# mpkuse/solve_keyframe_pose_graph

Measured on AMD Instinct MI355X. Metric: LM iters/sec + final chi2 vs Ceres, 100k-pose/300k-edge SE(3) graph, higher is better.
Workload: dtype f64

## Files before the change

solve_keyframe_pose_graph_amd/csrc/pgo_handle.hpp:

```cpp
#pragma once
#include <hip/hip_runtime.h>

#include <chrono>
#include <cstdlib>
#include <cstring>
#include <memory>
#include <string>
#include <thread>
#include <vector>

#include "pgo.h"
#include "pgo_internal.hpp"
#include "pgo_comm.hpp"
#include "pgo_mg_host.hpp"

#pragma GCC visibility push(hidden)
namespace pgo {

inline double now_s() { return std::chrono::duration<double>(std::chrono::steady_clock::now().time_since_epoch()).count(); }

inline bool debug_hooks_enabled() { static const bool on = []() { const char* e = std::getenv("PGO_ENABLE_DEBUG_HOOKS"); return e && e[0] == '1' && e[1] == 0; }(); return on; }
inline bool debug_poison() { static const bool on = []() { const char* e = std::getenv("PGO_DEBUG_POISON"); return debug_hooks_enabled() && e && e[0] == '1' && e[1] == 0; }(); return on; }
inline bool debug_break_coarse() { if (!debug_hooks_enabled()) return false; const char* e = std::getenv("PGO_DEBUG_BREAK_COARSE"); return e && e[0] == '1' && e[1] == 0; }

inline bool debug_no_split_update() { static const bool on = []() { const char* e = std::getenv("PGO_DEBUG_NO_SPLIT_UPDATE"); return debug_hooks_enabled() && e && e[0] == '1' && e[1] == 0; }(); return on; }
inline bool debug_split_hosts(int* a, int* b) {
    static const int v = []() {
        const char* e = std::getenv("PGO_DEBUG_SPLIT_HOSTS");
        if (!debug_hooks_enabled() || !e) return -1;
        char* end = nullptr; const long x = std::strtol(e, &end, 10);
        if (!end || *end != ',' || x < 0 || x > 63) return -1;
        const long y = std::strtol(end + 1, &end, 10);
        return (end && *end == 0 && y >= x && y <= 63) ? (int)(x * 64 + y) : -1;
    }();
    if (v < 0) return false;
    *a = v / 64; *b = v % 64;
    return true;
}

inline int debug_graph_after() {
    static const int v = []() {
        const char* e = std::getenv("PGO_DEBUG_GRAPH_AFTER");
        if (!debug_hooks_enabled() || !e) return 192;
        char* end = nullptr; const long n = std::strtol(e, &end, 10);
        return (end && *end == 0 && n >= 2 && n <= 1000000 && (n & 1) == 0) ? (int)n : 192;
    }();
    return v;
}

template <class T>
struct DBuf {
    T* p = nullptr;
    size_t cap = 0;
    DBuf() = default;
    DBuf(const DBuf&) = delete;
    DBuf& operator=(const DBuf&) = delete;
    ~DBuf() { if (p) (void)hipFree(p); }
    hipError_t ensure(size_t n) {
        if (n <= cap) return hipSuccess;
        if (p) { (void)hipFree(p); p = nullptr; cap = 0; }
        const size_t want = n + n / 8 + 64;
        hipError_t e = hipMalloc((void**)&p, want * sizeof(T));
        if (e == hipSuccess) cap = want;
        if (e == hipSuccess && debug_poison()) { e = hipMemset(p, 0xFF, want * sizeof(T)); if (e == hipSuccess) e = hipDeviceSynchronize(); }
        return e;
    }
    hipError_t upload(const std::vector<T>& v, hipStream_t st) {
        hipError_t e = ensure(v.empty() ? 1 : v.size());
        if (e == hipSuccess && !v.empty()) e = hipMemcpyAsync(p, v.data(), v.size() * sizeof(T), hipMemcpyHostToDevice, st);
        return e;
    }
};

struct EventPair {
    hipEvent_t e0 = nullptr, e1 = nullptr;
    hipError_t create() { hipError_t e = hipEventCreate(&e0); if (e == hipSuccess) e = hipEventCreate(&e1); return e; }
    ~EventPair() { if (e0) (void)hipEventDestroy(e0); if (e1) (void)hipEventDestroy(e1); }
};

struct HostClass {
    std::vector<int32_t> c1, c2, sw;
    std::vector<double> meas;
    std::vector<double> loss;
    int64_t size() const { return (int64_t)c1.size(); }
};

struct MgPrepared;
struct MgPreparedFree { void operator()(MgPrepared* Q) const; };
using MgImage = std::unique_ptr<MgPrepared, MgPreparedFree>;

struct LevelPlanDev { const int32_t* send_idx = nullptr; const int32_t* recv_idx = nullptr; const pgo_mg::ExchangePlan* plan = nullptr; };
struct SetupPlanDev { const int32_t* val_send = nullptr; const int32_t* val_dst = nullptr; const int32_t* val_sum_ptr = nullptr; const int32_t* val_sum_src = nullptr;
                      const int32_t* ps_send = nullptr; const int32_t* ps_recv = nullptr; const int32_t* rv_send = nullptr; const int32_t* rv_recv = nullptr; };
struct OwnRange { int64_t row0 = 0, row1 = 0, blk0 = 0, blk1 = 0, ps0 = 0, ps1 = 0, w0 = 0, w1 = 0, rT0 = 0, rT1 = 0; };

struct MgJob {
    enum Kind { none, fresh, regroup };
    Kind kind = none;
    std::thread thread;
    MgImage out;
    int rc = 0;
    MgImage old;
};

struct MgState {
    DBuf<double> f64; DBuf<int32_t> i32; DBuf<int64_t> i64;
    MgDev M{}; MgLevelDev levels[MG_MAX_LEVELS];
    bool fine = false; MgLevelDev fineF{}, fineT{};
    int fine_auto = -1;
    bool built = false, active = false;
    pgo_mg::BuildCache cache;
    std::vector<double> sw_built;
    int regroups = 0;
    uint64_t geometry_epoch = 0;
    MgJob job;
    std::vector<LevelPlanDev> lvl_plan;
    std::vector<pgo_mg::ExchangePlan> plans;
    std::vector<uint8_t> dist;
    pgo_mg::SetupPlans setup; int first_whole = 0;
    int32_t fw_row0 = 0, fw_row1 = 0; int64_t fw_blk0 = 0, fw_blk1 = 0;
    std::vector<SetupPlanDev> su_plan;
// ... 222 lines not shown
```

solve_keyframe_pose_graph_amd/csrc/pgo_kernels.hip:

```cpp
#include <algorithm>

#include "pgo_internal.hpp"

namespace pgo {

#ifndef PGO_NO_UNIFORM
__device__ __forceinline__ int wave_in_grid() { return __builtin_amdgcn_readfirstlane((int)(((int64_t)blockIdx.x * blockDim.x + threadIdx.x) >> 6)); }
__device__ __forceinline__ int wave_in_block() { return __builtin_amdgcn_readfirstlane((int)(threadIdx.x >> 6)); }
#else
__device__ __forceinline__ int wave_in_grid() { return (int)(((int64_t)blockIdx.x * blockDim.x + threadIdx.x) >> 6); }
__device__ __forceinline__ int wave_in_block() { return (int)(threadIdx.x >> 6); }
#endif

__device__ __forceinline__ double wave_sum(double v) {
#pragma unroll
    for (int o = 32; o > 0; o >>= 1) v += __shfl_down(v, o, 64);
    return v;
}
__device__ __forceinline__ double wave_max(double v) {
#pragma unroll
    for (int o = 32; o > 0; o >>= 1) v = fmax(v, __shfl_down(v, o, 64));
    return v;
}
#ifndef PGO_SERIAL_HEAD
__device__ __forceinline__ double strided_share(const double* __restrict__ p, int n) {
    constexpr int MAXK = 12;
    double v[MAXK];
#pragma unroll
    for (int k = 0; k < MAXK; ++k) { const int i = (int)threadIdx.x + k * (int)blockDim.x; v[k] = i < n ? p[i] : 0.0; }
    double s = 0.0;
#pragma unroll
    for (int k = 0; k < MAXK; ++k) s += v[k];
    for (int i = (int)threadIdx.x + MAXK * (int)blockDim.x; i < n; i += blockDim.x) s += p[i];
    return s;
}
#else
__device__ __forceinline__ double strided_share(const double* __restrict__ p, int n) { double s = 0.0; for (int i = threadIdx.x; i < n; i += blockDim.x) s += p[i]; return s; }
#endif
__device__ __forceinline__ double block_sum(double v, double* buf) {
    const int lane = threadIdx.x & 63, wave = threadIdx.x >> 6, nw = (blockDim.x + 63) >> 6;
    v = wave_sum(v);
    __syncthreads();
    if (lane == 0) buf[wave] = v;
    __syncthreads();
    double s = 0.0;
    if (threadIdx.x == 0) for (int i = 0; i < nw; ++i) s += buf[i];
    return s;
}
__device__ __forceinline__ double block_total(const double* __restrict__ partials, int n, double* buf) {
    double v = strided_share(partials, n);
    const int lane = threadIdx.x & 63, wave = threadIdx.x >> 6, nw = (blockDim.x + 63) >> 6;
    v = wave_sum(v);
    __syncthreads();
    if (lane == 0) buf[wave] = v;
    __syncthreads();
    double s = 0.0;
    for (int i = 0; i < nw; ++i) s += buf[i];
    return s;
}

__device__ __forceinline__ int pm(int r, int c) { return (c >> 1) * 12 + r * 2 + (c & 1); }

__device__ __forceinline__ void block_total2(const double* __restrict__ pa, int na, const double* __restrict__ pb, int nb, double* buf , double& sa, double& sb) {
    double va = strided_share(pa, na), vb = strided_share(pb, nb);
    const int lane = threadIdx.x & 63, wave = threadIdx.x >> 6, nw = (blockDim.x + 63) >> 6;
    va = wave_sum(va); vb = wave_sum(vb);
    __syncthreads();
    if (lane == 0) { buf[wave] = va; buf[nw + wave] = vb; }
    __syncthreads();
    sa = 0.0; sb = 0.0;
    for (int i = 0; i < nw; ++i) { sa += buf[i]; sb += buf[nw + i]; }
}

__device__ __forceinline__ void block_total3(const double* __restrict__ pa, int na, const double* __restrict__ pb, int nb, const double* __restrict__ pc, int nc, double* buf ,
                                             double& sa, double& sb, double& sc) {
    double va = strided_share(pa, na), vb = strided_share(pb, nb), vc = strided_share(pc, nc);
    const int lane = threadIdx.x & 63, wave = threadIdx.x >> 6, nw = (blockDim.x + 63) >> 6;
    va = wave_sum(va); vb = wave_sum(vb); vc = wave_sum(vc);
    __syncthreads();
    if (lane == 0) { buf[wave] = va; buf[nw + wave] = vb; buf[2 * nw + wave] = vc; }
    __syncthreads();
    sa = 0.0; sb = 0.0; sc = 0.0;
    for (int i = 0; i < nw; ++i) { sa += buf[i]; sb += buf[nw + i]; sc += buf[2 * nw + i]; }
// ... 1026 lines not shown
    return (int)g;
}
__global__ void cg_set_tolerance_kernel(CgDev C, double tol2) {
    if (threadIdx.x == 0 && blockIdx.x == 0) { C.scal[3] = tol2; if (!C.flags[1]) C.flags[0] = 0; }
}
void launch_cg_set_tolerance(const CgDev& C, double tol2, hipStream_t st) { hipLaunchKernelGGL(cg_set_tolerance_kernel, dim3(1), dim3(64), 0, st, C, tol2); }
__global__ void cg_poll_kernel(CgDev C, int32_t* __restrict__ hflags, double* __restrict__ hscal) {
    if (threadIdx.x < 3) { hflags[threadIdx.x] = C.flags[threadIdx.x]; hscal[threadIdx.x] = C.scal[threadIdx.x]; }
}
void launch_cg_poll(const CgDev& C, int32_t* host_flags, double* host_scal, hipStream_t st) { hipLaunchKernelGGL(cg_poll_kernel, dim3(1), dim3(64), 0, st, C, host_flags, host_scal); }

void launch_cg_init(const GraphDev& G, const CgDev& C, int warm, double tol2, hipStream_t st) {
    const int g = cg_grid(G);
    hipLaunchKernelGGL(cg_init_kernel, dim3(g), dim3(CG_BLOCK), 0, st, G, C, warm);
    hipLaunchKernelGGL(cg_scalars_init_kernel, dim3(1), dim3(256), 0, st, C, g, g, tol2);
}
void launch_cg_init_scalars(const CgDev& C, int nparts, int nparts_bb, double tol2, hipStream_t st) { hipLaunchKernelGGL(cg_scalars_init_kernel, dim3(1), dim3(256), 0, st, C, nparts, nparts_bb, tol2); }
int launch_cg_init_vectors(const GraphDev& G, const CgDev& C, int warm, hipStream_t st) {
    const int g = cg_grid(G);
    hipLaunchKernelGGL(cg_init_kernel, dim3(g), dim3(CG_BLOCK), 0, st, G, C, warm);
    return g;
}
void launch_cg_spmv(const GraphDev& G, const CgDev& C, int k, double tol2, hipStream_t st) {
    const int g = cg_grid(G);
    hipLaunchKernelGGL(cg_spmv_kernel, dim3(g), dim3(CG_BLOCK), 0, st, G, C, k & 1, k == 0 ? 1 : 0, g, tol2);
}
void launch_cg_update(const GraphDev& G, const CgDev& C, int k, int n_pq_partials, hipStream_t st) {
    const int g = cg_grid(G);
    hipLaunchKernelGGL(cg_update_kernel<false>, dim3(g), dim3(CG_BLOCK), 0, st, G, C, k & 1, n_pq_partials, g, 0);
}
void launch_cg_update_sr(const GraphDev& G, const CgDev& C, int k, int first, int n_pq_partials, hipStream_t st) {
    const int g = cg_grid(G);
    hipLaunchKernelGGL(cg_update_kernel<true>, dim3(g), dim3(CG_BLOCK), 0, st, G, C, k & 1, n_pq_partials, g, first);
}
void launch_cgcg_dots(const GraphDev& G, const CgDev& C, hipStream_t st) { hipLaunchKernelGGL(cgcg_dots_kernel, dim3(cg_grid(G)), dim3(CG_BLOCK), 0, st, G, C); }
void launch_cg_reduce2_live(const CgDev& C, const double* pa, int na, const double* pb, int nb, double* out, hipStream_t st) {
    hipLaunchKernelGGL(cg_reduce2_live_kernel, dim3(1), dim3(256), 0, st, C, pa, na, pb, nb, out);
}
void launch_cgcg_update(const GraphDev& G, const CgDev& C, int k, int first, hipStream_t st, const double* xq, const int32_t* sh_of, const double* two) {
    hipLaunchKernelGGL(cgcg_update_kernel, dim3(cg_grid(G)), dim3(CG_BLOCK), 0, st, G, C, k & 1, first, xq, sh_of, two);
}
void launch_cgcg_scalars_init(const CgDev& C, const double* bb_src, double tol2, hipStream_t st) { hipLaunchKernelGGL(cgcg_scalars_init_kernel, dim3(1), dim3(64), 0, st, C, bb_src, tol2); }
int cg_grid_size(const GraphDev& G) { return cg_grid(G); }
void launch_apply_operator(const GraphDev& G, const CgDev& C, const double* x, double* y, hipStream_t st) { hipLaunchKernelGGL(apply_operator_kernel, dim3(cg_grid(G)), dim3(CG_BLOCK), 0, st, G, C, x, y); }

template <bool LOSS>
__global__ __launch_bounds__(256) void mf_compact_kernel(GraphDev G, MfDev F, const double* __restrict__ pose8, const double* __restrict__ swv) {
    const int64_t i = (int64_t)blockIdx.x * blockDim.x + threadIdx.x;
    if (i >= F.ninc) return;
    const uint32_t ent = F.einc[i];
    const bool is_sw = (ent >> 31) != 0;
    const int64_t e = (ent & 0x7fffffffu) >> 1;
    const EdgeClassDev& C = is_sw ? G.sw : G.rel;
    const Pose P1 = load_pose_global(pose8, C.c1[e]);
    const Pose P2 = load_pose_global(pose8, C.c2[e]);
    const double* mp = C.meas + e;
    const size_t ep = (size_t)C.Epad;
    const Meas M{mp[0], mp[ep], mp[2 * ep], mp[3 * ep], mp[4 * ep], mp[5 * ep], mp[6 * ep], mp[7 * ep]};
    const double ws = is_sw ? swv[C.swidx[e]] : LOSS ? M.w * G.rel.lossc[e] : M.w;
    double rec[COMPACT_DOUBLES];
    edge_compact(P1, P2, M, ws, is_sw, rec);
    for (int pl = 0; pl < MF_PLANES; ++pl) F.rec[(size_t)pl * F.ninc_pad + i] = make_double2(rec[2 * pl], rec[2 * pl + 1]);
}

__device__ __forceinline__ double coarse_pending(const CoarseDev& K, const uint8_t* __restrict__ node_free, int64_t node, int r) {
    const double fr = node_free[node] ? 1.0 : 0.0;
    const double* y = K.yc + (size_t)(node / K.m) * 6;
    const double* d = K.d + (size_t)node * 3;
    const int c = r < 3 ? r : r - 3, c1 = c == 2 ? 0 : c + 1, c2 = c == 0 ? 2 : c - 1;
    const double yr = y[r], ya = y[c1], yb = y[c2], da = d[c1], db = d[c2];
    return fr * (r < 3 ? yr : yr - 2.0 * (da * yb - db * ya));
}

#ifdef PGO_MF_TIMELINE
__device__ unsigned long long pgo_mf_tl[MF_MAX_GRID * 16];
#define MF_TL(slot) do { __builtin_amdgcn_s_waitcnt(0); if (threadIdx.x == 0 && (slot) < 16) pgo_mf_tl[blockIdx.x * 16 + (slot)] = wall_clock64(); } while (0)
extern "C" int pgo_debug_mf_timeline(unsigned long long* out, int n) {
    return (int)hipMemcpyFromSymbol(out, HIP_SYMBOL(pgo_mf_tl), (size_t)n * sizeof(unsigned long long), 0, hipMemcpyDeviceToHost);
}
#else
#define MF_TL(slot) do {} while (0)
#endif

template <bool FUSED, bool COARSE = false>
#ifndef PGO_MF_WAVES
#define PGO_MF_WAVES 1
#endif
__global__ __launch_bounds__(MF_BLOCK, PGO_MF_WAVES) void mf_spmv_kernel(GraphDev G, MfDev F, ScaleDev Sc, CgDev C, const double* __restrict__ xin, double* __restrict__ yout,
                                                           int parity, int first, int nparts, double tol2, CoarseDev K = CoarseDev{}, int pending = 0) {
    __shared__ double contrib[MF_SLOTS * 7];
    __shared__ double pwin[MF_BLOCK];
    __shared__ double red[3 * (MF_BLOCK / 64) + 1];
    const int l = threadIdx.x;
    MF_TL(0);
    double beta = 0.0;
    const double* __restrict__ pprev = FUSED ? (parity ? C.p : C.p2) : xin;
    const double* __restrict__ z = FUSED ? C.z : xin;
    double v0_first = 0.0, v1_first = 0.0;
    int64_t i0_first = 0, i1_first = 0; int32_t n0_first = 0, n1_first = 0, sw_first = 0;
    {
        const int tile = blockIdx.x;
        if (tile < F.tiles) {
            i0_first = F.tile_inc0[tile]; i1_first = F.tile_inc0[tile + 1]; sw_first = F.tile_sw0[tile];
            const int32_t n0 = F.tile_node0[tile], n1 = F.tile_node0[tile + 1];
            n0_first = n0; n1_first = n1;
            if (l < (n1 - n0) * 6) {
                const size_t vi = (size_t)n0 * 6 + l;
                v0_first = z[vi];
                if (FUSED) v1_first = pprev[vi];
                if (COARSE && pending) { const double cp = coarse_pending(K, G.node_free, (int64_t)n0 + l / 6, l % 6); v0_first = K.m == 1 ? cp : v0_first + cp; }
            }
        }
    }
    if (!FUSED && first == 3) { if (cg_done(C)) return; }
    if (FUSED) {
        if (first) { if (cg_done(C)) return; }
        else {
            double rz_new, rz_old;
            bool coarse_negative = false;
            bool stopped;
            if (COARSE) {
                double rz_bj, rz_c;
                stopped = block_total3_done(C.flags, C.part_rz + parity * RZ_STRIDE, nparts, C.part_rz + parity * RZ_STRIDE + nparts, C.extra_rz, C.part_rz + (parity ^ 1) * RZ_STRIDE, nparts + C.extra_rz, red, rz_bj, rz_c, rz_old);
                rz_new = rz_bj + rz_c;
                coarse_negative = K.m != 1 && !(rz_new > C.scal[3] * C.scal[0]) && rz_bj > C.scal[3] * C.scal[0];
            } else stopped = block_total2_done(C.flags, C.part_rz + parity * RZ_STRIDE, nparts + C.extra_rz, C.part_rz + (parity ^ 1) * RZ_STRIDE, nparts + C.extra_rz, red, rz_new, rz_old);
            if (stopped) return;
            const bool breakdown = C.flags[1] != 0;
            if (breakdown || !(rz_new > C.scal[3] * C.scal[0])) {
                if (blockIdx.x == 0 && threadIdx.x == 0) { C.flags[0] = 1; if (!breakdown) { C.scal[1] = rz_new; if (coarse_negative || !(rz_new >= -C.scal[3] * C.scal[0])) C.flags[1] = 1; } }
                return;
            }
            beta = rz_new / rz_old;
            if (blockIdx.x == 0 && threadIdx.x == 0) C.scal[1] = rz_new;
        }
        if (blockIdx.x == 0 && threadIdx.x == 0) C.flags[2] += 1;
    }
    MF_TL(1);
    double* __restrict__ pcur = parity ? C.p2 : C.p;
    double pq = 0.0;
#ifdef PGO_MF_TIMELINE
    int tl_base = 2;
#endif
    for (int tile = blockIdx.x; tile < F.tiles; tile += gridDim.x) {
        const bool is_first = tile == (int)blockIdx.x;
        const int64_t i0 = is_first ? i0_first : F.tile_inc0[tile], i1 = is_first ? i1_first : F.tile_inc0[tile + 1];
        const int32_t n0 = is_first ? n0_first : F.tile_node0[tile], n1 = is_first ? n1_first : F.tile_node0[tile + 1];
        const int32_t swp = is_first ? sw_first : F.tile_sw0[tile];
        const int sw0 = swp & 0xffff, pair1 = (int)((uint32_t)swp >> 16);
        const int64_t i = i0 + l;
        const int nn = n1 - n0;
        MF_TL(tl_base + 0);
        if (l < nn * 6) {
            double v;
            if (COARSE) {
                const size_t vi = (size_t)n0 * 6 + l;
                double zf = v0_first;
                if (tile != (int)blockIdx.x) {
                    zf = z[vi];
                    if (pending) { const double cp = coarse_pending(K, G.node_free, (int64_t)n0 + l / 6, l % 6); zf = K.m == 1 ? cp : zf + cp; }
                }
                v = zf + beta * (tile == (int)blockIdx.x ? v1_first : pprev[vi]);
            } else if (tile == (int)blockIdx.x) v = FUSED ? v0_first + beta * v1_first : v0_first;
            else {
                const size_t vi = (size_t)n0 * 6 + l;
                v = z[vi];
                if (FUSED) v += beta * pprev[vi];
            }
            pwin[l] = v;
        }
        __syncthreads();
        MF_TL(tl_base + 1);
        if (i < i1) {
            const uint32_t ent = F.einc[i];
            const int32_t other = F.einc_other[i];
            const uint32_t sl = F.einc_slot[i];
            const bool is_sw = l >= sw0;
            const int side = (int)(ent & 1u);
            const int ownl = (int)(sl >> 18), slot_a = (int)(sl & 511u), slot_b = (int)((sl >> 9) & 511u);
            double rec[COMPACT_DOUBLES];
#pragma unroll
            for (int pl = 0; pl < 8; ++pl) { const double2 v = F.rec[(size_t)pl * F.ninc_pad + i]; rec[2 * pl] = v.x; rec[2 * pl + 1] = v.y; }
            double kscale = 0.0;
            if (is_sw) {
                {
                    const double q2c[4] = {-rec[0], -rec[1], -rec[2], rec[3]};
                    double dq[4];
                    quat_mul(q2c, rec + 4, dq);
                    rec[16] = rec[11]; rec[17] = rec[12]; rec[18] = rec[13];
                    rec[19] = 2.0 * dq[0]; rec[20] = 2.0 * dq[1]; rec[21] = 2.0 * dq[2];
                }
                kscale = sqrt(Sc.a_inv[(ent & 0x7fffffffu) >> 1]);
            } else {
#pragma unroll
                for (int k = 16; k < COMPACT_DOUBLES; ++k) rec[k] = 0.0;
            }
            MF_TL(tl_base + 2);
            double po[6], pt[6];
            {
                const double* a = pwin + ownl * 6;
#pragma unroll
                for (int c = 0; c < 6; ++c) po[c] = a[c];
            }
            if (other >= n0 && other < n1) {
                const double* b = pwin + (other - n0) * 6;
#pragma unroll
                for (int c = 0; c < 6; ++c) pt[c] = b[c];
            } else {
                const double2* b = reinterpret_cast<const double2*>(z + (size_t)other * 6);
                const double2 b0 = b[0], b1 = b[1], b2 = b[2];
                pt[0] = b0.x; pt[1] = b0.y; pt[2] = b1.x; pt[3] = b1.y; pt[4] = b2.x; pt[5] = b2.y;
                if (COARSE && pending) {
                    if (K.m == 1) {
#pragma unroll
                        for (int c = 0; c < 6; ++c) pt[c] = 0.0;
                    }
                    {
                        const double fr = G.node_free[other] ? 1.0 : 0.0;
                        const double* yy = K.yc + (size_t)(other / K.m) * 6;
                        const double* dd = K.d + (size_t)other * 3;
                        const double y0 = yy[0], y1 = yy[1], y2 = yy[2], y3 = yy[3], y4 = yy[4], y5 = yy[5], d0 = dd[0], d1 = dd[1], d2 = dd[2];
                        pt[0] += fr * y0; pt[1] += fr * y1; pt[2] += fr * y2;
                        pt[3] += fr * (y3 - 2.0 * (d1 * y2 - d2 * y1));
                        pt[4] += fr * (y4 - 2.0 * (d2 * y0 - d0 * y2));
                        pt[5] += fr * (y5 - 2.0 * (d0 * y1 - d1 * y0));
                    }
                }
                if (FUSED) {
                    const double2* c = reinterpret_cast<const double2*>(pprev + (size_t)other * 6);
                    const double2 c0 = c[0], c1 = c[1], c2 = c[2];
                    pt[0] += beta * c0.x; pt[1] += beta * c0.y; pt[2] += beta * c1.x; pt[3] += beta * c1.y; pt[4] += beta * c2.x; pt[5] += beta * c2.y;
                }
            }
            MF_TL(tl_base + 3);
            double y[6];
            if (l < pair1) {
                double y2[6];
                compact_apply_both(rec, po, pt, 0.0, y, y2);
#pragma unroll
                for (int r = 0; r < 6; ++r) contrib[slot_b * 7 + r] = y2[r];
            } else compact_apply(rec, side, po, pt, kscale, y);
#pragma unroll
            for (int r = 0; r < 6; ++r) contrib[slot_a * 7 + r] = y[r];
        }
        __syncthreads();
        MF_TL(tl_base + 4);
        if (l < nn * 6) {
            const int nl = l / 6, r = l - nl * 6;
            const int64_t node = (int64_t)n0 + nl;
            const size_t vi = (size_t)node * 6 + r;
            const double pr = pwin[l];
            const double lam = F.lam[vi];
            const uint8_t is_free = G.node_free[node];
            const ushort4 rg = F.node_rng[node];
            const int32_t pk = F.node_prior[node];
            double acc = lam * pr;
            MF_TL(tl_base + 5);
            if (is_free) {
                for (int j = rg.x; j < rg.y; ++j) acc += contrib[j * 7 + r];
                for (int j = rg.z; j < rg.w; ++j) acc += contrib[j * 7 + r];
                if (pk >= 0) {
                    const double* Jp = G.Jp + (size_t)pk * PRIOR_DOUBLES + 6;
                    double pn[6];
                    for (int c = 0; c < 6; ++c) pn[c] = pwin[nl * 6 + c];
                    double s = 0.0;
                    for (int ii = 0; ii < 6; ++ii) { double t = 0.0; for (int c = 0; c < 6; ++c) t += Jp[ii * 6 + c] * pn[c]; s += Jp[ii * 6 + r] * t; }
                    acc += s;
                }
            }
            if (FUSED) { pcur[vi] = pr; C.q[vi] = acc; pq += acc * pr; }
            else { yout[vi] = acc; pq += acc * pr; }
        }
        __syncthreads();
        MF_TL(tl_base + 6);
#ifdef PGO_MF_TIMELINE
        tl_base += 7;
#endif
    }
    if (FUSED || first >= 2) {
        const double s = block_sum(pq, red);
        if (threadIdx.x == 0) C.part_pq[blockIdx.x] = s;
    }
}

static inline int mf_grid(const MfDev& F) { const int g = F.tiles < MF_MAX_GRID ? F.tiles : MF_MAX_GRID; return g < 1 ? 1 : g; }
int mf_grid_size(const MfDev& F) { return mf_grid(F); }
void launch_mf_compact(const GraphDev& G, const MfDev& F, const double* pose8, const double* sw, hipStream_t st) {
    if (F.ninc <= 0) return;
    if (G.rel.lossc) hipLaunchKernelGGL(mf_compact_kernel<true>, dim3((unsigned)((F.ninc + 255) / 256)), dim3(256), 0, st, G, F, pose8, sw);
    else hipLaunchKernelGGL(mf_compact_kernel<false>, dim3((unsigned)((F.ninc + 255) / 256)), dim3(256), 0, st, G, F, pose8, sw);
}
void launch_mf_spmv(const GraphDev& G, const MfDev& F, const ScaleDev& Sc, const CgDev& C, int k, double tol2, hipStream_t st) {
    const int g = mf_grid(F);
    hipLaunchKernelGGL((mf_spmv_kernel<true, false>), dim3(g), dim3(MF_BLOCK), 0, st, G, F, Sc, C, (const double*)nullptr, (double*)nullptr, k & 1, k == 0 ? 1 : 0, cg_grid(G), tol2);
}
void launch_mf_spmv_coarse(const GraphDev& G, const MfDev& F, const ScaleDev& Sc, const CgDev& C, const CoarseDev& K, int k, double tol2, int nparts, int pending, hipStream_t st) {
    hipLaunchKernelGGL((mf_spmv_kernel<true, true>), dim3(mf_grid(F)), dim3(MF_BLOCK), 0, st, G, F, Sc, C, (const double*)nullptr, (double*)nullptr, k & 1, k == 0 ? 1 : 0, nparts, tol2, K, pending);
}
void launch_mf_apply_dot(const GraphDev& G, const MfDev& F, const ScaleDev& Sc, const CgDev& C, const double* x, double* y, hipStream_t st) {
    hipLaunchKernelGGL((mf_spmv_kernel<false, false>), dim3(mf_grid(F)), dim3(MF_BLOCK), 0, st, G, F, Sc, C, x, y, 0, 2, 0, 0.0);
}
void launch_mf_apply_dot_live(const GraphDev& G, const MfDev& F, const ScaleDev& Sc, const CgDev& C, hipStream_t st) {
    hipLaunchKernelGGL((mf_spmv_kernel<false, false>), dim3(mf_grid(F)), dim3(MF_BLOCK), 0, st, G, F, Sc, C, (const double*)C.z, C.q, 0, 3, 0, 0.0);
}
void launch_mf_apply(const GraphDev& G, const MfDev& F, const ScaleDev& Sc, const CgDev& C, const double* x, double* y, hipStream_t st) {
    hipLaunchKernelGGL((mf_spmv_kernel<false, false>), dim3(mf_grid(F)), dim3(MF_BLOCK), 0, st, G, F, Sc, C, x, y, 0, 1, 0, 0.0);
}

__global__ __launch_bounds__(256) void model_change_kernel(GraphDev G, LinDev L, ScaleDev Sc, const double* __restrict__ dp, double* __restrict__ ds_out, double* __restrict__ partials) {
    __shared__ double red[4];
    const int wave = threadIdx.x >> 6, lane = threadIdx.x & 63;
    const int tile_g = blockIdx.x * 4 + wave;
    const int ntile = G.rel.tiles + G.sw.tiles;
    double mc = 0.0;
    if (tile_g < ntile) {
        const bool is_sw = tile_g >= G.rel.tiles;
        const int tile = is_sw ? tile_g - G.rel.tiles : tile_g;
        const EdgeClassDev& C = is_sw ? G.sw : G.rel;
        const int64_t e = (int64_t)tile * TILE + lane;
        if (e < C.E) {
            const int32_t c1 = C.c1[e], c2 = C.c2[e];
            double d1[6], d2[6];
#pragma unroll
            for (int i = 0; i < 6; ++i) { d1[i] = dp[(size_t)c1 * 6 + i]; d2[i] = dp[(size_t)c2 * 6 + i]; }
            const int D = is_sw ? SW_DOUBLES : REL_DOUBLES;
            const double2* base = reinterpret_cast<const double2*>(C.J + tile_elem(D, e, 0));
            const int o1 = is_sw ? 7 : 3, o2 = is_sw ? 25 : 21;
            double u[7];
#pragma unroll
            for (int i = 0; i < 7; ++i) u[i] = 0.0;
#pragma unroll
            for (int row = 0; row < 6; ++row) {
#pragma unroll
                for (int kp = 0; kp < 3; ++kp) {
                    const double2 a = base[(o1 + row * 3 + kp) * TILE], b = base[(o2 + row * 3 + kp) * TILE];
                    u[row] += a.x * d1[2 * kp] + a.y * d1[2 * kp + 1] + b.x * d2[2 * kp] + b.y * d2[2 * kp + 1];
                }
            }
            double r[7];
            { double2 v; v = base[0]; r[0] = v.x; r[1] = v.y; v = base[TILE]; r[2] = v.x; r[3] = v.y; v = base[2 * TILE]; r[4] = v.x; r[5] = v.y; }
            r[6] = 0.0;
            if (is_sw) {
                double Js[7];
                { double2 v; v = base[3 * TILE]; r[6] = v.x; Js[0] = v.y; v = base[4 * TILE]; Js[1] = v.x; Js[2] = v.y;
                  v = base[5 * TILE]; Js[3] = v.x; Js[4] = v.y; v = base[6 * TILE]; Js[5] = v.x; Js[6] = v.y; }
                const double* cc = L.c + (size_t)e * 12;
                double acc = L.gs[e];
#pragma unroll
                for (int i = 0; i < 6; ++i) acc += cc[i] * d1[i] + cc[6 + i] * d2[i];
                const double ds = -acc * Sc.a_inv[e];
                ds_out[e] = ds;
#pragma unroll
                for (int i = 0; i < 7; ++i) u[i] += Js[i] * ds;
            }
#pragma unroll
            for (int i = 0; i < 7; ++i) mc += u[i] * (r[i] + 0.5 * u[i]);
        }
    }
    if (blockIdx.x == gridDim.x - 1) {
        for (int k = threadIdx.x; k < G.n_prior; k += blockDim.x) {
            const double* base = G.Jp + (size_t)k * PRIOR_DOUBLES;
            const int32_t node = G.prior[k].node;
            for (int row = 0; row < 6; ++row) {
                double u = 0.0;
                for (int c = 0; c < 6; ++c) u += base[6 + row * 6 + c] * dp[(size_t)node * 6 + c];
                mc += u * (base[row] + 0.5 * u);
            }
        }
// ... 1050 lines not shown
```

solve_keyframe_pose_graph_amd/csrc/pgo_measure.hip:

```cpp
#include <algorithm>
#include <cmath>
#include <cstring>
#include <vector>

#include "pgo_handle.hpp"

namespace {


int build_lm_system(pgo_problem* p) {
    const pgo_options& o = p->opt;
    if (!p->reuse_diagonal) launch_lm_diag(p->G, p->L, p->Sc, o.min_lm_diagonal, o.max_lm_diagonal, p->st);
    bool ok = true;
    return build_system(p, &ok);
}

int setup_block_jacobi(pgo_problem* p) {
    int rc;
    if ((rc = build_lm_system(p)) != PGO_OK) return rc;
    p->mg.active = false; p->coarse.active = false; p->C.extra_rz = 0;
    launch_cg_init(p->G, p->C, 0, 0.0, p->st);
    return PGO_OK;
}

// ... 55 lines not shown
    for (int l = 0; l + 1 < p->mg.M.n_levels; ++l) {
        const MgLevelDev& A = p->mg.levels[l];
        if (A.smoothed && A.rt_valf)
            cyc += (double)A.nnzb * (144.0 + 4.0) + 2.0 * (double)A.n_w * (144.0 + 4.0) + (double)A.n * (288.0 + 24.0 + 8.0 * 48.0 + 16.0) + (double)A.n_next * (288.0 + 2.0 * 48.0 + 8.0);
        else
            cyc += (A.smoothed ? 4.0 : 2.0) * (double)A.nnzb * (144.0 + 4.0) + (double)A.n * ((A.smoothed ? 4.0 : 2.0) * 288.0  + 24.0 + (A.smoothed ? 18.0 : 10.0) * 48.0 + 16.0);
    }
    cyc += (double)p->coarse.K.nc * (double)p->coarse.K.nc * 4.0 + (double)p->coarse.K.nc * 16.0;
    if (split_update) cyc += N * 48.0;
    return cyc;
}

double algorithmic_bytes(const pgo_problem* p, int which) {
    const GraphDev& G = p->G;
    const double N = (double)G.N, E = (double)(G.rel.E + G.sw.E), Es = (double)G.sw.E;
    switch (which) {
        case 0: return k1_algorithmic_bytes(G, true);
        case 1: return (624.0 * G.rel.E + 688.0 * Es) + 288.0 * E + 336.0 * N + 112.0 * Es;
        case 2: case 4: case 5: {
            const FineBytes fine = fine_iteration_bytes(p, choose_form(p, true).single_red());
            return which == 2 ? fine.matvec + fine.update : which == 4 ? fine.matvec : fine.update; }
        case 3: return k1_algorithmic_bytes(G, false);
        case 6: case 7: {
            if (p->local_ids) return (double)p->mg.blocks_own * 148.0 + (double)p->mg.rows_own * (288.0 + 24.0 + 8.0 * 48.0 + 16.0) + (double)p->coarse.K.nc * (double)p->coarse.K.nc * 4.0 + (double)p->coarse.K.nc * 16.0;
            const PcgForm f = multigrid_form(p, which);
            const double cyc = cycle_bytes(p, f.split.on());
            if (which == 7) return cyc;
            const FineBytes fine = fine_iteration_bytes(p, f.single_red());
            return fine.matvec + fine.update + cyc; }
        default: return 0.0;
    }
}

int time_launches(pgo_problem* p, int which, int launches, double* best_ms) {
    int rc;
    EventPair ev;
    HIPCHK(p, ev.create());
    const int turns = (p->comm && (which == 7 || which == 8)) ? p->world() : 1;
    const int batches = turns > 1 ? 3 : 1;
    *best_ms = -1.0;
    for (int turn = 0; turn < turns; ++turn) {
        if (turns > 1) {
            HIPCHK(p, hipStreamSynchronize(p->st));
            if (!p->comm->barrier()) { p->err = "in-process communicator: a rank left during pgo_time_kernel"; return PGO_ERR_COMM; }
            if (turn != p->rank()) continue;
        }
        for (int rep = 0; rep < 1 + batches; ++rep) {
            const int n = rep == 0 ? 1 : launches;
            if (rep >= 1) HIPCHK(p, hipEventRecord(ev.e0, p->st));
            for (int i = 0; i < n; ++i) if ((rc = enqueue(p, which, rep == 0 ? 0 : i + 1)) != PGO_OK) return rc;
            if (rep >= 1) HIPCHK(p, hipEventRecord(ev.e1, p->st));
            HIPCHK(p, hipStreamSynchronize(p->st));
            if (rep >= 1) { float msb = 0; HIPCHK(p, hipEventElapsedTime(&msb, ev.e0, ev.e1)); if (*best_ms < 0.0 || (double)msb < *best_ms) *best_ms = (double)msb; }
        }
    }
    if (turns > 1 && !p->comm->barrier()) { p->err = "in-process communicator: a rank left during pgo_time_kernel"; return PGO_ERR_COMM; }
    return PGO_OK;
}

}

extern "C" {

int pgo_time_kernel(pgo_problem* p, int32_t which, int32_t launches, double* avg_ms, double* algorithmic_bytes_out) {
    if (!p || launches <= 0 || !avg_ms) return PGO_ERR_INVALID_ARG;
    if (!p->in_solve) { p->err = "pgo_time_kernel needs an open solve (pgo_solve_begin)"; return PGO_ERR_STATE; }
    int rc;
    if ((rc = set_device(p)) != PGO_OK) return rc;
    if (which < 0 || which > 8) return PGO_ERR_INVALID_ARG;
    if (which == 5 && single_reduction(p)) {
        p->err = "pgo_time_kernel(5): the single-reduction update cannot be timed without its matvec; time the iteration (2) and the matvec (4) and subtract"; return PGO_ERR_STATE;
    }
    if ((which == 2 || which == 4 || which == 5) && (rc = setup_block_jacobi(p)) != PGO_OK) return rc;
    if (which >= 6 && (rc = setup_multigrid(p, which)) != PGO_OK) return rc;
    const double bytes = algorithmic_bytes(p, which);
    double best_ms = -1.0;
    if ((rc = time_launches(p, which, launches, &best_ms)) != PGO_OK) return rc;
    if (which == 8) { p->mg.active = false; if ((rc = build_mg(p)) != PGO_OK) return rc; }
    *avg_ms = best_ms / launches;
    if (algorithmic_bytes_out) *algorithmic_bytes_out = bytes;
    return PGO_OK;
}
int pgo_time_linearize_kernel(pgo_problem* p, int32_t launches, double* avg_ms, double* bytes) { return pgo_time_kernel(p, 0, launches, avg_ms, bytes); }

int pgo_time_vio_odometry_kernel(pgo_problem* p, int32_t f_max, int32_t launches, double* avg_ms, double* algorithmic_bytes) {
    if (!p || launches <= 0 || !avg_ms || f_max < 1) return PGO_ERR_INVALID_ARG;
    if (p->n_vio < 2) { p->err = "no resident VIO poses"; return PGO_ERR_STATE; }
    int rc;
    if ((rc = set_device(p)) != PGO_OK) return rc;
    std::vector<int32_t> c;
    for (int64_t u = 0; u < p->n_vio; ++u) for (int f = 1; f <= f_max; ++f) if (u - f >= 0) c.push_back((int32_t)u);
    const int64_t n = (int64_t)c.size();
    for (int64_t u = 0; u < p->n_vio; ++u) for (int f = 1; f <= f_max; ++f) if (u - f >= 0) c.push_back((int32_t)(u - f));
    DBuf<int32_t> d_c; DBuf<double> d_meas;
    HIPCHK(p, d_c.ensure((size_t)2 * n)); HIPCHK(p, d_meas.ensure((size_t)8 * n));
    HIPCHK(p, hipMemcpyAsync(d_c.p, c.data(), (size_t)2 * n * sizeof(int32_t), hipMemcpyHostToDevice, p->st));
    EventPair ev;
    HIPCHK(p, ev.create());
    const hipEvent_t e0 = ev.e0, e1 = ev.e1;
    launch_vio_odometry(n, d_c.p, d_c.p + n, p->d_vio.p, 1, d_meas.p, p->st);
    HIPCHK(p, hipEventRecord(e0, p->st));
    for (int i = 0; i < launches; ++i) launch_vio_odometry(n, d_c.p, d_c.p + n, p->d_vio.p, 1, d_meas.p, p->st);
    HIPCHK(p, hipEventRecord(e1, p->st));
    HIPCHK(p, hipStreamSynchronize(p->st));
    float ms = 0;
    HIPCHK(p, hipEventElapsedTime(&ms, e0, e1));
    *avg_ms = (double)ms / launches;
    if (algorithmic_bytes) *algorithmic_bytes = 128.0 * (double)p->n_vio + (8.0 + 64.0) * (double)n;
    return PGO_OK;
}

int pgo_dense_spd_inverse(pgo_problem* p, int32_t n, const double* a, double* a_inv, int32_t launches, double* avg_ms) {
    if (!p || n <= 0 || !a || !a_inv || launches < 1) return PGO_ERR_INVALID_ARG;
    int rc;
    if ((rc = set_device(p)) != PGO_OK) return rc;
    const int nc = (n + 63) / 64 * 64;
    std::vector<double> h((size_t)nc * nc, 0.0);
    for (int i = 0; i < nc; ++i) {
        if (i < n) std::memcpy(&h[(size_t)i * nc], a + (size_t)i * n, (size_t)n * sizeof(double));
        else h[(size_t)i * nc + i] = 1.0;
    }
    DBuf<double> d_a, d_scr; DBuf<int32_t> d_fail;
    HIPCHK(p, d_a.ensure((size_t)nc * nc)); HIPCHK(p, d_scr.ensure((size_t)nc * 64 + 4096)); HIPCHK(p, d_fail.ensure(1));
    CoarseDev K{}; K.nc = nc; K.Ac = d_a.p;
    EventPair ev;
    HIPCHK(p, ev.create());
    const hipEvent_t e0 = ev.e0, e1 = ev.e1;
    float total = 0;
    for (int l = 0; l < launches; ++l) {
        HIPCHK(p, hipMemcpyAsync(d_a.p, h.data(), h.size() * sizeof(double), hipMemcpyHostToDevice, p->st));
        HIPCHK(p, hipMemsetAsync(d_fail.p, 0, sizeof(int32_t), p->st));
        HIPCHK(p, hipEventRecord(e0, p->st));
        launch_coarse_invert(K, d_scr.p, d_fail.p, p->st);
        HIPCHK(p, hipEventRecord(e1, p->st));
        HIPCHK(p, hipStreamSynchronize(p->st));
        float ms = 0;
        HIPCHK(p, hipEventElapsedTime(&ms, e0, e1));
        total += ms;
    }
    int32_t fail = 1;
    HIPCHK(p, hipMemcpy(&fail, d_fail.p, sizeof(fail), hipMemcpyDeviceToHost));
    HIPCHK(p, hipMemcpy(h.data(), d_a.p, h.size() * sizeof(double), hipMemcpyDeviceToHost));
    for (int i = 0; i < n; ++i) std::memcpy(a_inv + (size_t)i * n, &h[(size_t)i * nc], (size_t)n * sizeof(double));
    if (avg_ms) *avg_ms = (double)total / launches;
    if (fail) { p->err = "matrix is not numerically positive definite"; return PGO_ERR_NUMERIC; }
    return PGO_OK;
}

int pgo_mg_level_norms(pgo_problem* p, int32_t level, double* out8) {
    if (!p || !out8) return PGO_ERR_INVALID_ARG;
    for (int k = 0; k < 8; ++k) out8[k] = 0.0;
    if (!p->mg.built || p->mg.fresh_pending() || level < 1 || level > p->mg.M.n_levels || (size_t)(level - 1) >= p->mg.own.size()) { p->err = "pgo_mg_level_norms: no such level (is a hierarchy installed?)"; return PGO_ERR_INVALID_ARG; }
    int rc;
    if ((rc = set_device(p)) != PGO_OK) return rc;
    const MgLevelDev& A = p->mg.levels[level - 1];
    const OwnRange& R = p->mg.own[(size_t)level - 1];
    HIPCHK(p, hipStreamSynchronize(p->st));
    auto sq64 = [&](const double* dev, int64_t first, int64_t count, double* out) -> int {
        if (!dev || count <= 0) return PGO_OK;
        std::vector<double> h((size_t)count);
        HIPCHK(p, hipMemcpy(h.data(), dev + first, (size_t)count * sizeof(double), hipMemcpyDeviceToHost));
        long double s = 0.0L; for (double v : h) s += (long double)v * v;
        *out = (double)s; return PGO_OK;
    };
    auto sq32 = [&](const float* dev, int64_t first, int64_t count, double* out) -> int {
        if (!dev || count <= 0) return PGO_OK;
// ... 104 lines not shown
```

Measured before the change: 118.1.

## Software-pipeline matrix-free SpMV tile loop with double-buffered window and prefetch

Measured after the change: 116.6. 0.987x the previous value.

```diff
diff --git a/solve_keyframe_pose_graph_amd/csrc/pgo_handle.hpp b/solve_keyframe_pose_graph_amd/csrc/pgo_handle.hpp
--- a/solve_keyframe_pose_graph_amd/csrc/pgo_handle.hpp
+++ b/solve_keyframe_pose_graph_amd/csrc/pgo_handle.hpp
@@ -37,6 +37,7 @@
     *a = v / 64; *b = v % 64;
     return true;
 }
+
 
 inline int debug_graph_after() {
     static const int v = []() {
diff --git a/solve_keyframe_pose_graph_amd/csrc/pgo_kernels.hip b/solve_keyframe_pose_graph_amd/csrc/pgo_kernels.hip
--- a/solve_keyframe_pose_graph_amd/csrc/pgo_kernels.hip
+++ b/solve_keyframe_pose_graph_amd/csrc/pgo_kernels.hip
@@ -1,4 +1,5 @@
 #include <algorithm>
+#include <cstdlib>
 
 #include "pgo_internal.hpp"
 
@@ -1191,6 +1192,9 @@
 #define MF_TL(slot) do {} while (0)
 #endif
 
+__device__ __forceinline__ int64_t uniform64(int64_t v) {
+    return (int64_t)(((uint64_t)(uint32_t)__builtin_amdgcn_readfirstlane((int)((uint64_t)v >> 32)) << 32) | (uint32_t)__builtin_amdgcn_readfirstlane((int)(uint32_t)v));
+}
 template <bool FUSED, bool COARSE = false>
 #ifndef PGO_MF_WAVES
 #define PGO_MF_WAVES 1
@@ -1198,30 +1202,38 @@
 __global__ __launch_bounds__(MF_BLOCK, PGO_MF_WAVES) void mf_spmv_kernel(GraphDev G, MfDev F, ScaleDev Sc, CgDev C, const double* __restrict__ xin, double* __restrict__ yout,
                                                            int parity, int first, int nparts, double tol2, CoarseDev K = CoarseDev{}, int pending = 0) {
     __shared__ double contrib[MF_SLOTS * 7];
-    __shared__ double pwin[MF_BLOCK];
+    __shared__ double pwin[2][MF_BLOCK];
     __shared__ double red[3 * (MF_BLOCK / 64) + 1];
+    __shared__ int s_stop;
+    constexpr bool PIPE = !COARSE, PF_WIN = PIPE && !FUSED;
     const int l = threadIdx.x;
     MF_TL(0);
     double beta = 0.0;
     const double* __restrict__ pprev = FUSED ? (parity ? C.p : C.p2) : xin;
     const double* __restrict__ z = FUSED ? C.z : xin;
-    double v0_first = 0.0, v1_first = 0.0;
-    int64_t i0_first = 0, i1_first = 0; int32_t n0_first = 0, n1_first = 0, sw_first = 0;
+    const bool head_free = !FUSED && first == 3;
+    int stop = 0;
+    if (head_free && l == 0) stop = C.flags[0];
+    int64_t i0 = 0, i1 = 0, i0_n = 0, i1_n = 0;
+    int32_t n0 = 0, n1 = 0, swp = 0, n0_n = 0, n1_n = 0, swp_n = 0;
+    double v0 = 0.0, v1 = 0.0;
+    uint32_t ent = 0; int32_t other = 0;
     {
-        const int tile = blockIdx.x;
+        const int tile = blockIdx.x, nxt = tile + (int)gridDim.x;
         if (tile < F.tiles) {
-            i0_first = F.tile_inc0[tile]; i1_first = F.tile_inc0[tile + 1]; sw_first = F.tile_sw0[tile];
-            const int32_t n0 = F.tile_node0[tile], n1 = F.tile_node0[tile + 1];
-            n0_first = n0; n1_first = n1;
+            i0 = F.tile_inc0[tile]; i1 = F.tile_inc0[tile + 1]; swp = F.tile_sw0[tile];
+            n0 = F.tile_node0[tile]; n1 = F.tile_node0[tile + 1];
+            if (PIPE && nxt < F.tiles) { i0_n = F.tile_inc0[nxt]; i1_n = F.tile_inc0[nxt + 1]; swp_n = F.tile_sw0[nxt]; n0_n = F.tile_node0[nxt]; n1_n = F.tile_node0[nxt + 1]; }
             if (l < (n1 - n0) * 6) {
                 const size_t vi = (size_t)n0 * 6 + l;
-                v0_first = z[vi];
-                if (FUSED) v1_first = pprev[vi];
-                if (COARSE && pending) { const double cp = coarse_pending(K, G.node_free, (int64_t)n0 + l / 6, l % 6); v0_first = K.m == 1 ? cp : v0_first + cp; }
-            }
-        }
-    }
-    if (!FUSED && first == 3) { if (cg_done(C)) return; }
+                v0 = z[vi];
+                if (FUSED) v1 = pprev[vi];
+                if (COARSE && pending) { const double cp = coarse_pending(K, G.node_free, (int64_t)n0 + l / 6, l % 6); v0 = K.m == 1 ? cp : v0 + cp; }
+            }
+            if (PIPE && i0 + l < i1) { ent = F.einc[i0 + l]; other = F.einc_other[i0 + l]; }
+        }
+    }
+    if (head_free && (int)blockIdx.x >= F.tiles) { if (cg_done(C)) return; }
     if (FUSED) {
         if (first) { if (cg_done(C)) return; }
         else {
@@ -1248,42 +1260,51 @@
     MF_TL(1);
     double* __restrict__ pcur = parity ? C.p2 : C.p;
     double pq = 0.0;
+    int buf = 0;
+    int64_t i0_v = 0, i1_v = 0; int32_t n0_v = 0, n1_v = 0, swp_v = 0;
 #ifdef PGO_MF_TIMELINE
     int tl_base = 2;
 #endif
     for (int tile = blockIdx.x; tile < F.tiles; tile += gridDim.x) {
         const bool is_first = tile == (int)blockIdx.x;
-        const int64_t i0 = is_first ? i0_first : F.tile_inc0[tile], i1 = is_first ? i1_first : F.tile_inc0[tile + 1];
-        const int32_t n0 = is_first ? n0_first : F.tile_node0[tile], n1 = is_first ? n1_first : F.tile_node0[tile + 1];
-        const int32_t swp = is_first ? sw_first : F.tile_sw0[tile];
+        const int nxt = tile + (int)gridDim.x, nxt2 = nxt + (int)gridDim.x;
+        if (!PIPE && !is_first) { i0 = uniform64(F.tile_inc0[tile]); i1 = uniform64(F.tile_inc0[tile + 1]); n0 = __builtin_amdgcn_readfirstlane(F.tile_node0[tile]); n1 = __builtin_amdgcn_readfirstlane(F.tile_node0[tile + 1]); swp = __builtin_amdgcn_readfirstlane(F.tile_sw0[tile]); }
         const int sw0 = swp & 0xffff, pair1 = (int)((uint32_t)swp >> 16);
         const int64_t i = i0 + l;
         const int nn = n1 - n0;
+        const bool row_lane = l < nn * 6, edge_lane = i < i1;
         MF_TL(tl_base + 0);
-        if (l < nn * 6) {
-            double v;
+        if (row_lane) {
+            if (!PF_WIN && !is_first) { v0 = z[(size_t)n0 * 6 + l]; if (FUSED) v1 = pprev[(size_t)n0 * 6 + l]; }
+            double v, cp = 0.0;
+            if (COARSE && pending && !is_first) cp = coarse_pending(K, G.node_free, (int64_t)n0 + l / 6, l % 6);
             if (COARSE) {
-                const size_t vi = (size_t)n0 * 6 + l;
-                double zf = v0_first;
-                if (tile != (int)blockIdx.x) {
-                    zf = z[vi];
-                    if (pending) { const double cp = coarse_pending(K, G.node_free, (int64_t)n0 + l / 6, l % 6); zf = K.m == 1 ? cp : zf + cp; }
-                }
-                v = zf + beta * (tile == (int)blockIdx.x ? v1_first : pprev[vi]);
-            } else if (tile == (int)blockIdx.x) v = FUSED ? v0_first + beta * v1_first : v0_first;
-            else {
-                const size_t vi = (size_t)n0 * 6 + l;
-                v = z[vi];
-                if (FUSED) v += beta * pprev[vi];
-            }
-            pwin[l] = v;
-        }
+                double zf = v0;
+                if (pending && !is_first) zf = K.m == 1 ? cp : zf + cp;
+                v = zf + beta * (FUSED ? v1 : is_first ? 0.0 : v0);
+            } else v = FUSED ? v0 + beta * v1 : v0;
+            pwin[buf][l] = v;
+        }
+        if (head_free && is_first && l == 0) s_stop = stop;
         __syncthreads();
+        if (head_free && is_first && __builtin_amdgcn_readfirstlane(s_stop) != 0) return;
         MF_TL(tl_base + 1);
-        if (i < i1) {
-            const uint32_t ent = F.einc[i];
-            const int32_t other = F.einc_other[i];
+        double v0_n = 0.0, v1_n = 0.0;
+        uint32_t ent_n = 0; int32_t other_n = 0;
+        if (PIPE && !is_first) {
+            i0_n = uniform64(i0_v); i1_n = uniform64(i1_v); n0_n = __builtin_amdgcn_readfirstlane(n0_v); n1_n = __builtin_amdgcn_readfirstlane(n1_v); swp_n = __builtin_amdgcn_readfirstlane(swp_v);
+        }
+        if (PIPE && nxt < F.tiles) {
+            if (PF_WIN && l < (n1_n - n0_n) * 6) {
+                const size_t vi = (size_t)n0_n * 6 + l;
+                v0_n = z[vi];
+                if (FUSED) v1_n = pprev[vi];
+            }
+            if (i0_n + l < i1_n) { ent_n = F.einc[i0_n + l]; other_n = F.einc_other[i0_n + l]; }
+        }
+        if (edge_lane) {
             const uint32_t sl = F.einc_slot[i];
+            if (!PIPE) { ent = F.einc[i]; other = F.einc_other[i]; }
             const bool is_sw = l >= sw0;
             const int side = (int)(ent & 1u);
             const int ownl = (int)(sl >> 18), slot_a = (int)(sl & 511u), slot_b = (int)((sl >> 9) & 511u);
@@ -1307,12 +1328,12 @@
             MF_TL(tl_base + 2);
             double po[6], pt[6];
             {
-                const double* a = pwin + ownl * 6;
+                const double* a = pwin[buf] + ownl * 6;
 #pragma unroll
                 for (int c = 0; c < 6; ++c) po[c] = a[c];
             }
             if (other >= n0 && other < n1) {
-                const double* b = pwin + (other - n0) * 6;
+                const double* b = pwin[buf] + (other - n0) * 6;
 #pragma unroll
                 for (int c = 0; c < 6; ++c) pt[c] = b[c];
             } else {
@@ -1354,24 +1375,25 @@
         }
         __syncthreads();
         MF_TL(tl_base + 4);
-        if (l < nn * 6) {
+        if (PIPE && nxt2 < F.tiles) { i0_v = F.tile_inc0[nxt2]; i1_v = F.tile_inc0[nxt2 + 1]; swp_v = F.tile_sw0[nxt2]; n0_v = F.tile_node0[nxt2]; n1_v = F.tile_node0[nxt2 + 1]; }
+        if (row_lane) {
             const int nl = l / 6, r = l - nl * 6;
             const int64_t node = (int64_t)n0 + nl;
             const size_t vi = (size_t)node * 6 + r;
-            const double pr = pwin[l];
+            const double pr = pwin[buf][l];
             const double lam = F.lam[vi];
             const uint8_t is_free = G.node_free[node];
             const ushort4 rg = F.node_rng[node];
             const int32_t pk = F.node_prior[node];
+            MF_TL(tl_base + 5);
             double acc = lam * pr;
-            MF_TL(tl_base + 5);
             if (is_free) {
                 for (int j = rg.x; j < rg.y; ++j) acc += contrib[j * 7 + r];
                 for (int j = rg.z; j < rg.w; ++j) acc += contrib[j * 7 + r];
                 if (pk >= 0) {
                     const double* Jp = G.Jp + (size_t)pk * PRIOR_DOUBLES + 6;
                     double pn[6];
-                    for (int c = 0; c < 6; ++c) pn[c] = pwin[nl * 6 + c];
+                    for (int c = 0; c < 6; ++c) pn[c] = pwin[buf][nl * 6 + c];
                     double s = 0.0;
                     for (int ii = 0; ii < 6; ++ii) { double t = 0.0; for (int c = 0; c < 6; ++c) t += Jp[ii * 6 + c] * pn[c]; s += Jp[ii * 6 + r] * t; }
                     acc += s;
@@ -1380,11 +1402,13 @@
             if (FUSED) { pcur[vi] = pr; C.q[vi] = acc; pq += acc * pr; }
             else { yout[vi] = acc; pq += acc * pr; }
         }
-        __syncthreads();
         MF_TL(tl_base + 6);
 #ifdef PGO_MF_TIMELINE
         tl_base += 7;
 #endif
+        if (PIPE) { i0 = i0_n; i1 = i1_n; n0 = n0_n; n1 = n1_n; swp = swp_n; }
+        v0 = v0_n; v1 = v1_n; ent = ent_n; other = other_n;
+        buf ^= 1;
     }
     if (FUSED || first >= 2) {
         const double s = block_sum(pq, red);
@@ -1392,7 +1416,16 @@
     }
 }
 
-static inline int mf_grid(const MfDev& F) { const int g = F.tiles < MF_MAX_GRID ? F.tiles : MF_MAX_GRID; return g < 1 ? 1 : g; }
+static inline int mf_grid_cap() {
+    static const int cap = []() {
+        const char* m = std::getenv("PGO_ENABLE_DEBUG_HOOKS"); const char* e = std::getenv("PGO_DEBUG_MF_GRID");
+        if (!m || m[0] != '1' || m[1] != 0 || !e) return MF_MAX_GRID;
+        char* end = nullptr; const long n = std::strtol(e, &end, 10);
+        return (end && end != e && *end == 0 && n >= 1 && n <= MF_MAX_GRID) ? (int)n : MF_MAX_GRID;
+    }();
+    return cap;
+}
+static inline int mf_grid(const MfDev& F) { const int cap = mf_grid_cap(), g = F.tiles < cap ? F.tiles : cap; return g < 1 ? 1 : g; }
 int mf_grid_size(const MfDev& F) { return mf_grid(F); }
 void launch_mf_compact(const GraphDev& G, const MfDev& F, const double* pose8, const double* sw, hipStream_t st) {
     if (F.ninc <= 0) return;
diff --git a/solve_keyframe_pose_graph_amd/csrc/pgo_measure.hip b/solve_keyframe_pose_graph_amd/csrc/pgo_measure.hip
--- a/solve_keyframe_pose_graph_amd/csrc/pgo_measure.hip
+++ b/solve_keyframe_pose_graph_amd/csrc/pgo_measure.hip
@@ -161,6 +161,13 @@
     return PGO_OK;
 }
 int pgo_time_linearize_kernel(pgo_problem* p, int32_t launches, double* avg_ms, double* bytes) { return pgo_time_kernel(p, 0, launches, avg_ms, bytes); }
+
+int pgo_debug_mf_grid(pgo_problem* p, int32_t* tiles, int32_t* workgroups) {
+    if (!p || !tiles || !workgroups) return PGO_ERR_INVALID_ARG;
+    if (!p->built_mf) { p->err = "pgo_debug_mf_grid: this graph has no matrix-free operator"; return PGO_ERR_STATE; }
+    *tiles = p->F.tiles; *workgroups = mf_grid_size(p->F);
+    return PGO_OK;
+}
 
 int pgo_time_vio_odometry_kernel(pgo_problem* p, int32_t f_max, int32_t launches, double* avg_ms, double* algorithmic_bytes) {
     if (!p || launches <= 0 || !avg_ms || f_max < 1) return PGO_ERR_INVALID_ARG;
```
